# olegroshka/vae-channel-dynamics

Measured on AMD Instinct MI355X. Metric: images/sec SDXL-VAE train step @256x256 (tracking on), higher is better.
Workload: dtype f32

## Files before the change

vae-channel-dynamics_amd/csrc/bf16_frag.h:

```cpp
#pragma once
#include "common.h"

typedef __bf16 bf16x8 __attribute__((ext_vector_type(8)));
typedef __bf16 bf16x4 __attribute__((ext_vector_type(4)));
typedef short s16x4 __attribute__((ext_vector_type(4)));
typedef short s16x8 __attribute__((ext_vector_type(8)));
typedef unsigned short u16;

__device__ __forceinline__ uint2 pack4(f32x4 v) {
  bf16x4 h;
#pragma unroll
  for (int e = 0; e < 4; ++e) h[e] = (__bf16)v[e];
  return __builtin_bit_cast(uint2, h);
}
__device__ __forceinline__ f32x4 unpack4(uint2 r) {
  f32x4 v;
  v[0] = __builtin_bit_cast(float, r.x << 16);
  v[1] = __builtin_bit_cast(float, r.x & 0xffff0000u);
  v[2] = __builtin_bit_cast(float, r.y << 16);
  v[3] = __builtin_bit_cast(float, r.y & 0xffff0000u);
  return v;
}
__device__ __forceinline__ uint4 buf_load4_raw(__amdgpu_buffer_rsrc_t rs, unsigned esize, int eoff) {
  return __builtin_bit_cast(uint4, __builtin_amdgcn_raw_buffer_load_b128(rs, eoff >= 0 ? (unsigned)eoff * esize : BUF_OOB, 0, 0));
}
__device__ __forceinline__ f32x4 raw4_to_f32(uint4 r, bool bf) {
  if (bf) return unpack4(uint2{r.x, r.y});
  return __builtin_bit_cast(f32x4, r);
}
__device__ __forceinline__ float buf_load1_elem(__amdgpu_buffer_rsrc_t rs, bool bf, int eoff) {
  if (bf) return __builtin_bit_cast(float, (unsigned)__builtin_amdgcn_raw_buffer_load_b16(rs, eoff >= 0 ? (unsigned)eoff * 2u : BUF_OOB, 0, 0) << 16);
  return __builtin_bit_cast(float, __builtin_amdgcn_raw_buffer_load_b32(rs, eoff >= 0 ? (unsigned)eoff * 4u : BUF_OOB, 0, 0));
}
__device__ __forceinline__ void buf_store1_elem(__amdgpu_buffer_rsrc_t rs, bool bf, int eoff, float v) {
  if (bf) {
    const __bf16 h = (__bf16)v;
    __builtin_amdgcn_raw_buffer_store_b16(__builtin_bit_cast(unsigned short, h), rs, eoff >= 0 ? (unsigned)eoff * 2u : BUF_OOB, 0, 0);
  } else {
    __builtin_amdgcn_raw_buffer_store_b32(__builtin_bit_cast(unsigned, v), rs, eoff >= 0 ? (unsigned)eoff * 4u : BUF_OOB, 0, 0);
  }
}
__device__ __forceinline__ bf16x8 frag_direct(const u16* p) {
  return __builtin_bit_cast(bf16x8, *reinterpret_cast<const uint4*>(p));
}
__device__ __forceinline__ bf16x8 frag_tr(const u16* p, int ld) {
  typedef __attribute__((address_space(3))) s16x4 lds_s16x4;
  const s16x4 lo = __builtin_amdgcn_ds_read_tr16_b64_v4i16((lds_s16x4*)(p));
  const s16x4 hi = __builtin_amdgcn_ds_read_tr16_b64_v4i16((lds_s16x4*)(p + 4 * ld));
  s16x8 r = {lo[0], lo[1], lo[2], lo[3], hi[0], hi[1], hi[2], hi[3]};
  return __builtin_bit_cast(bf16x8, r);
}
```

vae-channel-dynamics_amd/csrc/igemm.hip:

```cpp
#include "bf16_frag.h"
#include <algorithm>
#include <stdlib.h>
#include <type_traits>

#include "launchers.h"

namespace {

struct LanePos {
  int lr, lh, trq, trp, trh;
};
__device__ __forceinline__ LanePos lane_pos(int lane) { return LanePos{lane & 31, lane >> 5, (lane & 15) >> 2, lane & 3, (lane >> 4) & 1}; }

struct F32 {
  typedef float elem;
  typedef f32x4 raw4;
  typedef f32x4 frag;
  typedef unsigned off_t;
  static constexpr int BK_ROWS = 32, BK_WGRAD = 32;
  static constexpr int KG = 8;
  static constexpr int PAD_K = 4, PAD_T = 4;
  static constexpr bool SETPRIO = true;
  static constexpr bool PAIR16 = false;
  static constexpr int PLANES = 1;
  static constexpr bool LDS_DYNAMIC = false;
  static constexpr bool flag(int32_t) { return false; }

  static __device__ __forceinline__ raw4 load4(__amdgpu_buffer_rsrc_t rs, unsigned, bool ok, int row, int ld, int c) {
    return VAE_BUF_LOAD4(rs, oob_unless(ok, ((unsigned)row * (unsigned)ld + (unsigned)c) * 4u));
  }
  static __device__ __forceinline__ f32x4 to_f32(raw4 r, bool) { return r; }
  static __device__ __forceinline__ void put4(elem* d, f32x4 v, int) { *reinterpret_cast<f32x4*>(d) = v; }
  static __device__ __forceinline__ void put4_stored(elem* d, raw4, f32x4 v, bool, int) { put4(d, v, 0); }
  static __device__ __forceinline__ frag frag_k(const elem* p, int) { return *reinterpret_cast<const f32x4*>(p); }
  static __device__ __forceinline__ frag frag_t(const elem* tile, int ld, int kg, LanePos l, int col0, int) {
    frag v;
#pragma unroll
    for (int j = 0; j < 4; ++j) v[j] = tile[(kg * 8 + l.lh * 4 + j) * ld + col0 + l.lr];
    return v;
  }
  template <int MI, int NI>
  static __device__ __forceinline__ void frags_tt(frag* a, frag* b, const elem* sA, int ldA, int colA, const elem* sB, int ldB, int colB, int kg, LanePos l,
                                                  int, int) {
#pragma unroll
    for (int j = 0; j < 4; ++j) {
      const int k = kg * 8 + l.lh * 4 + j;
#pragma unroll
      for (int mi = 0; mi < MI; ++mi) a[mi][j] = sA[k * ldA + colA + mi * 32 + l.lr];
#pragma unroll
      for (int ni = 0; ni < NI; ++ni) b[ni][j] = sB[k * ldB + colB + ni * 32 + l.lr];
    }
  }
  template <int MI, int NI>
  static __device__ __forceinline__ void mma(f32x16 (&acc)[MI][NI], const frag* a, const frag* b) {
#pragma unroll
    for (int j = 0; j < 4; ++j)
#pragma unroll
      for (int mi = 0; mi < MI; ++mi)
#pragma unroll
        for (int ni = 0; ni < NI; ++ni) acc[mi][ni] = __builtin_amdgcn_mfma_f32_32x32x2f32(a[mi][j], b[ni][j], acc[mi][ni], 0, 0, 0);
  }
  static __device__ __forceinline__ off_t out_off(bool ok, int orow, int ldc, int col) {
    return ok ? ((unsigned)orow * (unsigned)ldc + (unsigned)col) * 4u : BUF_OOB;
  }
  static __device__ __forceinline__ bool inside(off_t o) { return o != BUF_OOB; }
  static __device__ __forceinline__ float load1(__amdgpu_buffer_rsrc_t rs, bool, off_t o) {
    return __builtin_bit_cast(float, __builtin_amdgcn_raw_buffer_load_b32(rs, o, 0, 0));
  }
  static __device__ __forceinline__ void store1(__amdgpu_buffer_rsrc_t rs, bool, off_t o, float v) {
    __builtin_amdgcn_raw_buffer_store_b32(__builtin_bit_cast(unsigned, v), rs, o, 0, 0);
  }
};

struct BF16 {
  typedef u16 elem;
  typedef uint4 raw4;
  typedef bf16x8 frag;
  typedef int off_t;
  static constexpr int BK_ROWS = 64, BK_WGRAD = 32;
  static constexpr int KG = 16;
  static constexpr int PAD_K = 8, PAD_T = 32;
  static constexpr bool SETPRIO = false;
  static constexpr bool PAIR16 = true;
  static constexpr int PLANES = 1;
  static constexpr bool LDS_DYNAMIC = false;
  static __device__ __forceinline__ bool flag(int32_t v) { return v != 0; }

  static __device__ __forceinline__ raw4 load4(__amdgpu_buffer_rsrc_t rs, unsigned esize, bool ok, int row, int ld, int c) {
    return buf_load4_raw(rs, esize, neg_unless(ok, row * ld + c));
  }
  static __device__ __forceinline__ f32x4 to_f32(raw4 r, bool bf) { return raw4_to_f32(r, bf); }
  static __device__ __forceinline__ void put4(elem* d, f32x4 v, int) { *reinterpret_cast<uint2*>(d) = pack4(v); }
  static __device__ __forceinline__ void put4_stored(elem* d, raw4 r, f32x4 v, bool bf, int) {
    *reinterpret_cast<uint2*>(d) = bf ? uint2{r.x, r.y} : pack4(v);
  }
  static __device__ __forceinline__ frag frag_k(const elem* p, int) { return frag_direct(p); }
  static __device__ __forceinline__ frag frag_t(const elem* tile, int ld, int kg, LanePos l, int col0, int) {
    return frag_tr(tile + (kg * 16 + l.lh * 8 + l.trq) * ld + col0 + l.trh * 16 + l.trp * 4, ld);
  }
  template <int MI, int NI>
  static __device__ __forceinline__ void frags_tt(frag* a, frag* b, const elem* sA, int ldA, int colA, const elem* sB, int ldB, int colB, int kg, LanePos l,
                                                  int, int) {
#pragma unroll
    for (int mi = 0; mi < MI; ++mi) a[mi] = frag_t(sA, ldA, kg, l, colA + mi * 32, 0);
#pragma unroll
    for (int ni = 0; ni < NI; ++ni) b[ni] = frag_t(sB, ldB, kg, l, colB + ni * 32, 0);
  }
  template <int MI, int NI>
  static __device__ __forceinline__ void mma(f32x16 (&acc)[MI][NI], const frag* a, const frag* b) {
#pragma unroll
    for (int mi = 0; mi < MI; ++mi)
#pragma unroll
      for (int ni = 0; ni < NI; ++ni) acc[mi][ni] = __builtin_amdgcn_mfma_f32_32x32x16_bf16(a[mi], b[ni], acc[mi][ni], 0, 0, 0);
  }
  static __device__ __forceinline__ off_t out_off(bool ok, int orow, int ldc, int col) { return ok ? orow * ldc + col : -1; }
  static __device__ __forceinline__ bool inside(off_t o) { return o >= 0; }
  static __device__ __forceinline__ float load1(__amdgpu_buffer_rsrc_t rs, bool bf, off_t o) { return buf_load1_elem(rs, bf, o); }
  static __device__ __forceinline__ void store1(__amdgpu_buffer_rsrc_t rs, bool bf, off_t o, float v) { buf_store1_elem(rs, bf, o, v); }

  static __device__ __forceinline__ bool pair16(const vae_igemm_args& p, bool cbf, bool rbf, const char* C) {
    return cbf && (p.N % 2 == 0) && (p.ldc % 2 == 0) && (p.res == nullptr || rbf) && p.track == nullptr && ((reinterpret_cast<uintptr_t>(C) & 3u) == 0);
  }
  template <int MI, int NI, class RowPixel>
  static __device__ __forceinline__ void store_pairs(const vae_igemm_args& p, const f32x16 (&acc)[MI][NI], int ni, __amdgpu_buffer_rsrc_t rsC,
                                                     __amdgpu_buffer_rsrc_t rsR, int col, bool colok, int m0, int trow0, int lh, bool s2c,
                                                     RowPixel row_pixel) {
    const bool odd = col & 1;
    const float b0 = (p.bias && colok) ? p.bias[col & ~1] : 0.f, b1 = (p.bias && colok) ? p.bias[col | 1] : 0.f;
#pragma unroll
    for (int mi = 0; mi < MI; ++mi) {
      unsigned o16[8], rr[8];
#pragma unroll
      for (int j = 0; j < 8; ++j) {
        const int r = 2 * j + (odd ? 1 : 0);
        const int row = trow0 + mi * 32 + (r & 3) + 8 * (r >> 2) + 4 * lh;
        int orow = row;
        if (s2c) {
          int b, y, x;
          row_pixel(row < p.M ? row : m0, b, y, x);
          orow = (b * p.g.Ho + y) * p.g.Wo + x;
        }
        o16[j] = (colok && row < p.M) ? (unsigned)(orow * p.ldc + (col & ~1)) * 2u : BUF_OOB;
        rr[j] = 0u;
      }
      if (p.res) {
#pragma unroll
        for (int j = 0; j < 8; ++j) rr[j] = __builtin_amdgcn_raw_buffer_load_b32(rsR, o16[j], 0, 0);
      }
#pragma unroll
      for (int j = 0; j < 8; ++j) {
        const float a0 = p.alpha * acc[mi][ni][2 * j], a1 = p.alpha * acc[mi][ni][2 * j + 1];
        const float recv = lane_xor1(odd ? a0 : a1);
        typedef __bf16 bf16x2_t __attribute__((ext_vector_type(2)));
        bf16x2_t h;
        h[0] = (__bf16)((odd ? recv : a0) + b0 + __builtin_bit_cast(float, rr[j] << 16));
        h[1] = (__bf16)((odd ? a1 : recv) + b1 + __builtin_bit_cast(float, rr[j] & 0xffff0000u));
        __builtin_amdgcn_raw_buffer_store_b32(__builtin_bit_cast(unsigned, h), rsC, o16[j], 0, 0);
      }
    }
  }
};

#ifndef VAE_FLAT_X3
#define VAE_FLAT_X3 1
#endif
struct F32X3 : F32 {
  typedef u16 elem;
  struct frag { bf16x8 p[3]; };
  static constexpr int BK_ROWS = 16, BK_WGRAD = 16;
  static constexpr int KG = 16;
  static constexpr int PAD_K = 8, PAD_T = 32;
  static constexpr bool SETPRIO = false;
  static constexpr int PLANES = 3;
  static constexpr bool LDS_DYNAMIC = true;

  static __device__ __forceinline__ void put4(elem* d, f32x4 v, int ps) {
    const uint2 hi = pack4(v);
    const f32x4 h = unpack4(hi);
    f32x4 r;
#pragma unroll
    for (int e = 0; e < 4; ++e) r[e] = v[e] - h[e];
    const uint2 mid = pack4(r);
    const f32x4 m = unpack4(mid);
#pragma unroll
    for (int e = 0; e < 4; ++e) r[e] = r[e] - m[e];
    *reinterpret_cast<uint2*>(d) = hi;
    *reinterpret_cast<uint2*>(d + ps) = mid;
    *reinterpret_cast<uint2*>(d + 2 * ps) = pack4(r);
  }
  static __device__ __forceinline__ void put4_stored(elem* d, raw4, f32x4 v, bool, int ps) { put4(d, v, ps); }
  static __device__ __forceinline__ frag frag_k(const elem* p, int ps) {
    frag f;
#pragma unroll
    for (int q = 0; q < 3; ++q) f.p[q] = BF16::frag_k(p + q * ps, 0);
    return f;
  }
  static __device__ __forceinline__ frag frag_t(const elem* tile, int ld, int kg, LanePos l, int col0, int ps) {
    frag f;
#pragma unroll
    for (int q = 0; q < 3; ++q) f.p[q] = BF16::frag_t(tile + q * ps, ld, kg, l, col0, 0);
    return f;
  }
  template <int MI, int NI>
  static __device__ __forceinline__ void frags_tt(frag* a, frag* b, const elem* sA, int ldA, int colA, const elem* sB, int ldB, int colB, int kg, LanePos l,
                                                  int psA, int psB) {
#pragma unroll
    for (int mi = 0; mi < MI; ++mi) a[mi] = frag_t(sA, ldA, kg, l, colA + mi * 32, psA);
#pragma unroll
    for (int ni = 0; ni < NI; ++ni) b[ni] = frag_t(sB, ldB, kg, l, colB + ni * 32, psB);
  }
  template <int MI, int NI>
  static __device__ __forceinline__ void mma(f32x16 (&acc)[MI][NI], const frag* a, const frag* b) {
    constexpr int PA[6] = {0, 2, 1, 0, 1, 0}, PB[6] = {2, 0, 1, 1, 0, 0};
#pragma unroll
    for (int t = 0; t < 6; ++t)
#pragma unroll
      for (int mi = 0; mi < MI; ++mi)
#pragma unroll
        for (int ni = 0; ni < NI; ++ni)
          acc[mi][ni] = __builtin_amdgcn_mfma_f32_32x32x16_bf16(a[mi].p[PA[t]], b[ni].p[PB[t]], acc[mi][ni], 0, 0, 0);
  }
};

template <bool VEC, int WAVES>
using F32For = std::conditional_t<VEC && WAVES == 8 && (VAE_FLAT_X3 != 0), F32X3, F32>;

template <class P, int BM, int BN, bool BKM, int XF>
constexpr int rows_lds_elems() {
  constexpr int BK = P::BK_ROWS;
  return 2 * P::PLANES * (BM * (BK + P::PAD_K) + (BKM ? BK * (BN + P::PAD_T) : BN * (BK + P::PAD_K))) +
         ((XF != VAE_XF_NONE) ? 2 * SS_HALF * (4 / (int)sizeof(typename P::elem)) : 0);
}
template <class P, int BM, int BN, int XF>
constexpr int wgrad_lds_elems() {
  return 2 * P::PLANES * P::BK_WGRAD * (BM + P::PAD_T + BN + P::PAD_T) + ((XF != VAE_XF_NONE) ? 2 * SS_HALF * (4 / (int)sizeof(typename P::elem)) : 0);
}
extern __shared__ __attribute__((aligned(16))) unsigned char lds_dynamic[];

template <int MI, int NI>
__device__ __forceinline__ void zero_acc(f32x16 (&acc)[MI][NI]) {
#pragma unroll
  for (int mi = 0; mi < MI; ++mi)
#pragma unroll
    for (int ni = 0; ni < NI; ++ni)
#pragma unroll
      for (int r = 0; r < 16; ++r) acc[mi][ni][r] = 0.f;
}

template <class P, int BM, int BN, int WM, int WN, bool BKM, bool VEC, int XF>
__device__ __forceinline__ void rows_body(const vae_igemm_args& p) {
  typedef typename P::elem elem;
  constexpr int BK = P::BK_ROWS;
  constexpr int NT = 64 * WM * WN;
  constexpr int KQ = BK / 4;
  constexpr int RP = NT / KQ;
  constexpr int LDA = BK + P::PAD_K;
  constexpr int LDB = BKM ? (BN + P::PAD_T) : (BK + P::PAD_K);
  constexpr int SA = BM * LDA;
  constexpr int SB = BKM ? BK * LDB : BN * LDB;
  constexpr int PL = P::PLANES;
  constexpr int STAGE = PL * (SA + SB);
  constexpr int SS = (XF != VAE_XF_NONE) ? 2 * SS_HALF * (4 / (int)sizeof(elem)) : 0;
  constexpr int TM = BM / WM, TN = BN / WN, MI = TM / 32, NI = TN / 32;
  constexpr int AR = BM / RP;
  constexpr int NQ = BN / 4, KR = NT / NQ;
  constexpr int BR = BKM ? (BK / KR) : (BN / RP);
  static_assert(AR >= 1 && BR >= 1 && TM % 32 == 0 && TN % 32 == 0 && (BK / P::KG == 1 || BK / P::KG == 2 || BK / P::KG == 4), "tile/wave layout");
  static_assert(2 * STAGE + SS == rows_lds_elems<P, BM, BN, BKM, XF>(), "the launcher reserves what the body lays out");
  __shared__ __attribute__((aligned(16))) elem smem_static[P::LDS_DYNAMIC ? 1 : 2 * STAGE + SS];
  elem* const smem = P::LDS_DYNAMIC ? reinterpret_cast<elem*>(lds_dynamic) : smem_static;
  float* sS = reinterpret_cast<float*>(smem + 2 * STAGE);

  const int tid = threadIdx.x, lane = tid & 63, wave = tid >> 6;
  const int wm = wave / WN, wn = wave % WN;
  const LanePos lp = lane_pos(lane);
  const int lr = lp.lr, lh = lp.lh;
  const int tilesN = (p.N + BN - 1) / BN;
  const int tm = blockIdx.x / tilesN, tn = blockIdx.x % tilesN;
  const int m0 = tm * BM, n0 = tn * BN;
  const int z = blockIdx.z;
  const vae_conv_geom g = p.g;
  const SrcMap smap = make_srcmap(g);
  const bool abf = P::flag(p.a_bf16), cbf = P::flag(p.out_bf16), rbf = P::flag(p.res_bf16);
  const unsigned esA = abf ? 2u : 4u;
  const char* __restrict__ A = reinterpret_cast<const char*>(p.A) + (int64_t)z * p.sAb * esA;
  const float* __restrict__ W = p.W + (int64_t)z * p.sWb;
  const int hw = g.Ho * g.Wo;

  const bool s2c = (g.mode == VAE_MODE_DGRAD_S2);
  const int hh = g.Ho >> 1, wh = g.Wo >> 1;
  const int cls_rows = s2c ? p.M >> 2 : 1;
  const int cls = s2c ? m0 / cls_rows : 0;
  const int cpy = cls >> 1, cpx = cls & 1;
  const int nkw = s2c ? (cpx ? 1 : 2) : 3;
  const int ntaps = s2c ? (cpy ? 1 : 2) * nkw : g.taps;
  auto row_pixel = [&](int m, int& b, int& y, int& x) {
    if (s2c) {
      const int r = m - cls * cls_rows;
      b = r / (hh * wh);
      const int rem = r - b * (hh * wh);
      const int i = rem / wh;
      y = 2 * i + cpy;
      x = 2 * (rem - i * wh) + cpx;
    } else {
      b = m / hw;
      const int rem = m - b * hw;
      y = rem / g.Wo;
      x = rem - y * g.Wo;
    }
  };

  const int b_base = s2c ? (m0 - cls * cls_rows) / (hh * wh) : m0 / hw;
  const size_t img = (size_t)g.Hs * g.Ws * g.Cs;
  const size_t abytes = (size_t)(g.B - b_base) * img * esA, wbytes = (size_t)(BKM ? (int64_t)p.K * p.sk : (int64_t)p.N * p.sn) * 4u;
  const auto rsA = VAE_BUF_RSRC(A + (int64_t)b_base * img * esA, abytes < BUF_MAX ? abytes : BUF_MAX);
  const auto rsW = VAE_BUF_RSRC(W, wbytes < BUF_MAX ? wbytes : BUF_MAX);

  const int k4 = tid % KQ, r0 = tid / KQ;
  const int n4 = tid % NQ, kq = tid / NQ;
  int rb[AR], ry[AR], rx[AR];
#pragma unroll
  for (int i = 0; i < AR; ++i) {
    const int m = m0 + r0 + RP * i;
    if (m < p.M) {
      row_pixel(m, rb[i], ry[i], rx[i]);
    } else {
      rb[i] = -1; ry[i] = 0; rx[i] = 0;
    }
  }

  const int b_lo = m0 / hw;
  if (XF != VAE_XF_NONE) {
    const int b_hi = (min(p.M, m0 + BM) - 1) / hw;
    const int nent = min((b_hi - b_lo + 1) * p.K, SS_HALF);
    for (int i = tid; i < nent; i += NT) {
      const int j = i / p.K, c = i - j * p.K;
      sS[i] = p.scale[(int64_t)(b_lo + j) * g.Cs + c];
      sS[SS_HALF + i] = p.shift[(int64_t)(b_lo + j) * g.Cs + c];
    }
  }

  f32x16 acc[MI][NI];
  zero_acc(acc);

  const int kchunks = (p.K + BK - 1) / BK;
  const int steps = ntaps * kchunks;

  typename P::raw4 ra[AR];
  f32x4 rw[BR];
  int a_b[AR];
  int reg_c0 = 0;

  auto load_regs = [&](int s) {
    const int ord = s / kchunks;
    const int c0 = (s - ord * kchunks) * BK;
    reg_c0 = c0;
    int kh, kw;
    if (s2c) {
      const int a = ord / nkw;
      kh = cpy ? 1 : 2 * a;
      kw = cpx ? 1 : 2 * (ord - a * nkw);
    } else {
      kh = (g.taps == 9) ? ord / 3 : 0;
      kw = (g.taps == 9) ? ord - kh * 3 : 0;
    }
    const int tap = kh * 3 + kw;
    const int c = c0 + k4 * 4;
#pragma unroll
    for (int i = 0; i < AR; ++i) {
      int sy = 0, sx = 0;
      const bool ok = src_pixel(smap, ry[i], rx[i], kh, kw, sy, sx) && (rb[i] >= 0);
      if constexpr (VEC) ra[i] = P::load4(rsA, esA, ok && c < p.K, ((rb[i] - b_base) * g.Hs + sy) * g.Ws + sx, g.Cs, c);
      else ra[i] = load4s(p.A + (int64_t)z * p.sAb + (((int64_t)rb[i] * g.Hs + sy) * g.Ws + sx) * g.Cs + c, ok, c, p.K);
      a_b[i] = ok ? rb[i] : -1;
    }
    if (!BKM) {
#pragma unroll
      for (int i = 0; i < BR; ++i) {
        const int n = n0 + r0 + RP * i;
        if constexpr (VEC) rw[i] = VAE_BUF_LOAD4(rsW, oob_unless(n < p.N && c < p.K, ((unsigned)n * (unsigned)p.sn + (unsigned)tap * (unsigned)p.st + (unsigned)c) * 4u));
        else rw[i] = load4s(W + (int64_t)n * p.sn + (int64_t)tap * p.st + c, n < p.N, c, p.K);
      }
    } else {
#pragma unroll
      for (int i = 0; i < BR; ++i) {
        const int k = c0 + kq + KR * i;
        const int n = n0 + n4 * 4;
        if constexpr (VEC) rw[i] = VAE_BUF_LOAD4(rsW, oob_unless(k < p.K && n < p.N, ((unsigned)k * (unsigned)p.sk + (unsigned)tap * (unsigned)p.st + (unsigned)n) * 4u));
        else rw[i] = load4s(W + (int64_t)k * p.sk + (int64_t)tap * p.st + n, k < p.K, n, p.N);
      }
    }
  };
  auto store_lds = [&](elem* sA, elem* sB) {
    const int c = reg_c0 + k4 * 4;
#pragma unroll
    for (int i = 0; i < AR; ++i) {
      f32x4 v = P::to_f32(ra[i], abf);
      if (XF != VAE_XF_NONE) {
        const bool ok = (a_b[i] >= 0) && (c < p.K);
        const int o = ok ? (a_b[i] - b_lo) * p.K + c : 0;
        v = xform4_tab<XF>(v, sS + o, sS + SS_HALF + o, ok);
      }
      P::put4(&sA[(r0 + RP * i) * LDA + k4 * 4], v, SA);
    }
#pragma unroll
    for (int i = 0; i < BR; ++i) {
      if (!BKM) P::put4(&sB[(r0 + RP * i) * LDB + k4 * 4], rw[i], SB);
      else P::put4(&sB[(kq + KR * i) * LDB + n4 * 4], rw[i], SB);
    }
  };
  typename P::frag fa[2][MI], fb[2][NI];
  auto fetch = [&](const elem* sA, const elem* sB, int kg, typename P::frag* a, typename P::frag* b) {
#pragma unroll
    for (int mi = 0; mi < MI; ++mi) a[mi] = P::frag_k(&sA[(wm * TM + mi * 32 + lr) * LDA + kg * P::KG + lh * (P::KG / 2)], SA);
#pragma unroll
    for (int ni = 0; ni < NI; ++ni) {
      if (!BKM) b[ni] = P::frag_k(&sB[(wn * TN + ni * 32 + lr) * LDB + kg * P::KG + lh * (P::KG / 2)], SB);
      else b[ni] = P::frag_t(sB, LDB, kg, lp, wn * TN + ni * 32, SB);
    }
  };
  constexpr int NKG = BK / P::KG;
  auto compute = [&](const elem* sA, const elem* sB, int kg) {
    if (kg + 1 < NKG) fetch(sA, sB, kg + 1, fa[(kg + 1) & 1], fb[(kg + 1) & 1]);
    __builtin_amdgcn_sched_barrier(0);
    if (P::SETPRIO) __builtin_amdgcn_s_setprio(1);
    P::mma(acc, fa[kg & 1], fb[kg & 1]);
    if (P::SETPRIO) __builtin_amdgcn_s_setprio(0);
    __builtin_amdgcn_sched_barrier(0);
  };
  load_regs(0);
  __syncthreads();
  store_lds(smem, smem + PL * SA);
  if (steps > 1) load_regs(1);
  __syncthreads();
  for (int s = 0; s < steps; ++s) {
    const elem* cA = smem + (s & 1) * STAGE;
    const elem* cB = cA + PL * SA;
    fetch(cA, cB, 0, fa[0], fb[0]);
    if (NKG > 1) compute(cA, cB, 0);
    if (NKG == 4) compute(cA, cB, 1);
    if (s + 1 < steps) {
      elem* nA = smem + ((s + 1) & 1) * STAGE;
      store_lds(nA, nA + PL * SA);
      if (s + 2 < steps) load_regs(s + 2);
    }
    compute(cA, cB, NKG / 2);
    if (NKG == 4) compute(cA, cB, 3);
    __syncthreads();
  }

  const unsigned esC = cbf ? 2u : 4u, esR = rbf ? 2u : 4u;
  char* __restrict__ C = reinterpret_cast<char*>(p.C) + (int64_t)z * p.sCb * esC;
  const auto rsC = VAE_BUF_RSRC(C, (size_t)p.M * p.ldc * esC);
  const auto rsR = VAE_BUF_RSRC(p.res ? reinterpret_cast<const char*>(p.res) + (int64_t)z * p.sCb * esR : C, (size_t)p.M * p.ldc * (p.res ? esR : esC));
  float tsum[NI];
#pragma unroll
  for (int ni = 0; ni < NI; ++ni) tsum[ni] = 0.f;
  bool pair16 = false;
  if constexpr (P::PAIR16) pair16 = P::pair16(p, cbf, rbf, C);
#pragma unroll
  for (int ni = 0; ni < NI; ++ni) {
    const int col = n0 + wn * TN + ni * 32 + lr;
    const bool colok = col < p.N;
    const float bv = (p.bias && colok) ? p.bias[col] : 0.f;
    if constexpr (P::PAIR16) {
      if (pair16) {
        P::store_pairs(p, acc, ni, rsC, rsR, col, colok, m0, m0 + wm * TM, lh, s2c, row_pixel);
        continue;
      }
    }
#pragma unroll
    for (int mi = 0; mi < MI; ++mi) {
      typename P::off_t off[16];
      float rv[16];
#pragma unroll
      for (int r = 0; r < 16; ++r) {
        const int row = m0 + wm * TM + mi * 32 + (r & 3) + 8 * (r >> 2) + 4 * lh;
        int orow = row;
        if (s2c) {
          int b, y, x;
          row_pixel(row < p.M ? row : m0, b, y, x);
          orow = (b * g.Ho + y) * g.Wo + x;
        }
        off[r] = P::out_off(colok && row < p.M, orow, p.ldc, col);
        rv[r] = 0.f;
      }
      if (p.res) {
#pragma unroll
        for (int r = 0; r < 16; ++r) rv[r] = P::load1(rsR, rbf, off[r]);
      }
#pragma unroll
      for (int r = 0; r < 16; ++r) {
        const float v = p.alpha * acc[mi][ni][r] + bv + rv[r];
        P::store1(rsC, cbf, off[r], v);
        tsum[ni] += P::inside(off[r]) ? fabsf(v) : 0.f;
      }
    }
  }
  if (p.track && z == 0) {
    float* red = reinterpret_cast<float*>(smem);
#pragma unroll
    for (int ni = 0; ni < NI; ++ni) {
      const float s2 = tsum[ni] + __shfl_xor(tsum[ni], 32, 64);
      if (lh == 0) red[wm * BN + wn * TN + ni * 32 + lr] = s2;
    }
    __syncthreads();
    if (tid < BN) {
      float t = 0.f;
#pragma unroll
      for (int w = 0; w < WM; ++w) t += red[w * BN + tid];
      if (n0 + tid < p.N) p.track[(int64_t)tm * p.N + n0 + tid] = t;
    }
  }
}

template <class P, int BM, int BN, int WM, int WN, bool VEC, int XF>
__device__ __forceinline__ void wgrad_body(const vae_wgrad_args& p) {
  typedef typename P::elem elem;
  constexpr int BK = P::BK_WGRAD;
  constexpr int NT = 64 * WM * WN;
  constexpr int LDA = BM + P::PAD_T, LDB = BN + P::PAD_T;
  constexpr int SA = BK * LDA, SB = BK * LDB;
  constexpr int PL = P::PLANES;
// ... 513 lines not shown
```

vae-channel-dynamics_amd/csrc/wgrad3_wino.hip:

```cpp
#include "wino_common.h"
#ifndef VAE_ABLATE
#define VAE_ABLATE 0
#endif
#ifndef VAE_WGRAD_DEFER
#define VAE_WGRAD_DEFER 2
#endif
#ifndef VAE_WGRAD_PRIO
#define VAE_WGRAD_PRIO 1
#endif
#include <algorithm>
#include <type_traits>

namespace {

constexpr int GCI = 32, GCO = 128, GNT = 512;
constexpr int XS = 20;
constexpr int SXF = 4 * GCI * XS;
constexpr int SYF = 2 * GCO * XS;
constexpr int GSTAGE = SXF + SYF;

template <int XF>
__global__ __launch_bounds__(GNT, 1) void wgrad3_wino_kernel(vae_wgrad_args p, int strips, int64_t nunits) {
  __shared__ __attribute__((aligned(16))) float smem[2 * GSTAGE];

  const int tid = threadIdx.x, lane = tid & 63, wave = tid >> 6;
  const int lr = lane & 31, lh = lane >> 5;
  const vae_conv_geom g = p.g;
  const int tilesN = p.N / GCI, ntile = tilesN * (p.M / GCO);
  const wino::SplitTile wg = wino::split_tile_of_workgroup<true>(blockIdx.x, p.nsplit, ntile);
  const int tile = wg.tile, split = wg.split;
  const int tm = tile / tilesN, tn = tile % tilesN;
  const int m0 = tm * GCO, n0 = tn * GCI;
  const wino::UnitRange ur = wino::unit_range(nunits, p.nsplit, split);
  const int64_t ubeg = ur.ubeg;
  const int nu = ur.nu;
  const int upi = (g.Ho / 2) * strips;
  const bool do_bias = (p.bias_partial != nullptr) && tn == 0;
#ifdef VAE_WGRAD_TIMING
  constexpr int TS0 = 2, TSN = 8;
  const bool tw = (tid & 255) == 0 && blockIdx.x < 8 && p.out != nullptr;
  unsigned long long* const tout = reinterpret_cast<unsigned long long*>(p.out) + (blockIdx.x * 2 + (tid >> 8)) * (4 + TSN * 5);
  unsigned long long tst[5];
  const unsigned long long te0 = __builtin_amdgcn_s_memtime(), tr0 = __builtin_amdgcn_s_memrealtime();
#define GSTAMP(i) do { __builtin_amdgcn_sched_barrier(0); tst[i] = __builtin_amdgcn_s_memtime(); __builtin_amdgcn_sched_barrier(0); } while (0)
#define GSTAMPS_OUT(k) do { if (tw && (k) >= TS0 && (k) < TS0 + TSN) { _Pragma("unroll") for (int i_ = 0; i_ < 5; ++i_) tout[4 + ((k) - TS0) * 5 + i_] = tst[i_]; } } while (0)
#else
#define GSTAMP(i) do { } while (0)
#define GSTAMPS_OUT(k) do { } while (0)
#endif

  const int xx = tid & 15, xq = (tid >> 4) & 7, xr = tid >> 7;
  const bool xe_role = tid < 128 && (tid & 8) == 0;
  const int ex = 16 + (tid & 1), er = (tid >> 1) & 3;
  const int yq = tid >> 4;
  const auto rsX = VAE_BUF_RSRC(p.X, (size_t)g.B * g.Hs * g.Ws * g.Cs * 4u);
  const auto rsY = VAE_BUF_RSRC(p.dY, (size_t)g.B * g.Ho * g.Wo * p.ldy * 4u);
  struct Stg {
    f32x4 rx, rxe, ry[2];
    int b;
    bool xin, xein;
  };
  const f32x4 z4 = {0.f, 0.f, 0.f, 0.f};
  Stg s0{z4, z4, {z4, z4}, -1, false, false}, s1 = s0;
  f32x4 bsum = z4;
  f32x4 rsc = {1.f, 1.f, 1.f, 1.f}, rsh = z4;
  int sc_b = -1;
  int ub = (int)(ubeg / upi), uty = (int)((ubeg - (int64_t)ub * upi) / strips), ustrip = (int)((ubeg - (int64_t)ub * upi) % strips);
  const unsigned thrX = ((xr * g.Ws + xx) * g.Cs + n0 + 4 * xq) * 4u, thrE = ((er * g.Ws + ex) * g.Cs + n0 + 4 * xq) * 4u;
  const unsigned thrY = (xx * p.ldy + m0 + 4 * yq) * 4u, rowY = (unsigned)g.Wo * p.ldy * 4u;
  const int tfX = (xr == 0 ? 1 : 0) | (xr == 3 ? 2 : 0) | (xx == 0 ? 4 : 0) | 16;
  const int tfE = xe_role ? ((er == 0 ? 1 : 0) | (er == 3 ? 2 : 0) | (ex == 17 ? 8 : 0) | 16) : 31;
  auto load_unit = [&](int k, Stg& r) {
    const bool ok = k < nu;
    const int b = ub, ty = uty, x0 = ustrip * 16;
    if (++ustrip == strips) {
      ustrip = 0;
      if (++uty == g.Ho / 2) {
        uty = 0;
        ++ub;
      }
    }
    r.b = ok ? b : -1;
    const int uf = (ty == 0 ? 1 : 0) | (2 * ty + 2 >= g.Hs ? 2 : 0) | (x0 == 0 ? 4 : 0) | (x0 + 16 >= g.Ws ? 8 : 0) | (ok ? 0 : 16);
    const unsigned baseX = (unsigned)((b * g.Hs + 2 * ty - 1) * g.Ws + x0 - 1) * (unsigned)g.Cs * 4u;
    const unsigned baseY = (unsigned)((b * g.Ho + 2 * ty) * g.Wo + x0) * (unsigned)p.ldy * 4u;
    r.xin = (tfX & uf) == 0;
    r.rx = VAE_BUF_LOAD4(rsX, r.xin ? baseX + thrX : BUF_OOB);
    r.xein = (tfE & uf) == 0;
    r.rxe = VAE_BUF_LOAD4(rsX, r.xein ? baseX + thrE : BUF_OOB);
#pragma unroll
    for (int a = 0; a < 2; ++a) r.ry[a] = VAE_BUF_LOAD4(rsY, ok ? baseY + a * rowY + thrY : BUF_OOB);
  };
  auto xform = [&](f32x4 v, bool in) {
    if (XF != VAE_XF_NONE) {
#pragma unroll
      for (int e = 0; e < 4; ++e) {
        float u = v[e] * rsc[e] + rsh[e];
        if (XF == VAE_XF_AFFINE_SILU) u = silu_f(u);
        v[e] = in ? u : 0.f;
      }
    }
    return v;
  };
  auto store_unit = [&](float* st, const Stg& r) {
    float* sx = st;
    float* sy = st + SXF;
    if (XF != VAE_XF_NONE && r.b >= 0 && r.b != sc_b) {
      sc_b = r.b;
      rsc = *reinterpret_cast<const f32x4*>(p.scale + (int64_t)sc_b * g.Cs + n0 + 4 * xq);
      rsh = *reinterpret_cast<const f32x4*>(p.shift + (int64_t)sc_b * g.Cs + n0 + 4 * xq);
    }
    const f32x4 v = xform(r.rx, r.xin);
#pragma unroll
    for (int e = 0; e < 4; ++e) sx[(xr * GCI + 4 * xq + e) * XS + xx] = v[e];
    if (xe_role) {
      const f32x4 ve = xform(r.rxe, r.xein);
#pragma unroll
      for (int e = 0; e < 4; ++e) sx[(er * GCI + 4 * xq + e) * XS + ex] = ve[e];
    }
#pragma unroll
    for (int a = 0; a < 2; ++a) {
#pragma unroll
      for (int e = 0; e < 4; ++e) sy[(a * GCO + 4 * yq + e) * XS + xx] = r.ry[a][e];
      if (do_bias) bsum += r.ry[a];
    }
  };

  const int wi = wave >> 1, jh = wave & 1;
  const int vr1 = wi == 0 ? 0 : (wi == 2 ? 2 : 1), vr2 = wi == 0 ? 2 : (wi == 1 ? 2 : (wi == 2 ? 1 : 3));
  const int voff1 = (vr1 * GCI + lr) * XS + 8 * lh, voff2 = (vr2 * GCI + lr) * XS + 8 * lh;
  const int dr1 = wi == 3 ? 1 : 0;

  f32x16 acc[2][4];
#pragma unroll
  for (int pi = 0; pi < 2; ++pi)
#pragma unroll
    for (int nb = 0; nb < 4; ++nb)
#pragma unroll
      for (int e = 0; e < 16; ++e) acc[pi][nb][e] = 0.f;

  load_unit(0, s0);
  store_unit(smem, s0);
  load_unit(1, s1);
  __syncthreads();

  auto run = [&](auto WI, auto JH) {
    constexpr int wic = decltype(WI)::value, jhc = decltype(JH)::value;
    constexpr bool two = wic == 1 || wic == 2;
    constexpr bool vplus = wic == 1;
    constexpr int ndef = wic >= 2 ? VAE_WGRAD_DEFER : 0;
    static_assert(ndef >= 0 && ndef <= 2, "bb holds the operands of two channel blocks");
    f32x4 a4[2], bb[2][2];
    if (ndef > 0) {
      a4[0] = a4[1] = z4;
      bb[0][0] = bb[0][1] = bb[1][0] = bb[1][1] = z4;
    }
    auto held_back = [&]() {
#pragma unroll
      for (int e = 0; e < 4; ++e)
#pragma unroll
        for (int nb = 4 - ndef; nb < 4; ++nb)
#pragma unroll
          for (int pi = 0; pi < 2; ++pi) acc[pi][nb] = __builtin_amdgcn_mfma_f32_32x32x2f32(a4[pi][e], bb[nb & 1][pi][e], acc[pi][nb], 0, 0, 0);
    };
    auto step = [&](int k, const Stg& cur, Stg& nxt) {
      const float* cx = smem + (k & 1) * GSTAGE;
      const float* cy = cx + SXF;
      float* nst = smem + ((k + 1) & 1) * GSTAGE;
      GSTAMP(0);
      if (ndef > 0) {
        __builtin_amdgcn_sched_barrier(0);
        held_back();
        __builtin_amdgcn_sched_barrier(0);
      }
      GSTAMP(1);
      f32x4 rd[2][2];
      auto read_d = [&](int nb, f32x4 (&d)[2][2]) {
        const int doff = (dr1 * GCO + nb * 32 + lr) * XS + 8 * lh;
#pragma unroll
        for (int c = 0; c < 2; ++c) {
          d[0][c] = *reinterpret_cast<const f32x4*>(&cy[doff + 4 * c]);
          if (two) d[1][c] = *reinterpret_cast<const f32x4*>(&cy[doff + GCO * XS + 4 * c]);
        }
      };
      auto build_b = [&](const f32x4 (&d)[2][2], f32x4 (&b4)[2]) {
        float rc[8];
#pragma unroll
        for (int c = 0; c < 2; ++c)
#pragma unroll
          for (int e = 0; e < 4; ++e) rc[4 * c + e] = !two ? d[0][c][e] : (vplus ? d[0][c][e] + d[1][c][e] : d[0][c][e] - d[1][c][e]);
#pragma unroll
        for (int e = 0; e < 4; ++e) {
          if (jhc == 0) {
            b4[0][e] = rc[2 * e];
            b4[1][e] = rc[2 * e] + rc[2 * e + 1];
          } else {
            b4[0][e] = rc[2 * e] - rc[2 * e + 1];
            b4[1][e] = rc[2 * e + 1];
          }
        }
      };
      {
        f32x4 u1[3], u2[3];
#pragma unroll
        for (int c = 0; c < 3; ++c) {
          u1[c] = *reinterpret_cast<const f32x4*>(&cx[voff1 + 4 * c]);
          u2[c] = *reinterpret_cast<const f32x4*>(&cx[voff2 + 4 * c]);
        }
        float rc[12];
#pragma unroll
        for (int c = 0; c < 3; ++c)
#pragma unroll
          for (int e = 0; e < 4; ++e) rc[4 * c + e] = vplus ? u1[c][e] + u2[c][e] : u1[c][e] - u2[c][e];
        __builtin_amdgcn_sched_barrier(0);
        read_d(0, rd);
#pragma unroll
        for (int e = 0; e < 4; ++e) {
          if (jhc == 0) {
            a4[0][e] = rc[2 * e] - rc[2 * e + 2];
            a4[1][e] = rc[2 * e + 1] + rc[2 * e + 2];
          } else {
            a4[0][e] = rc[2 * e + 2] - rc[2 * e + 1];
            a4[1][e] = rc[2 * e + 1] - rc[2 * e + 3];
          }
        }
        build_b(rd, bb[0]);
        read_d(1, rd);
      }
      if (!(VAE_ABLATE & 2) && wave < 4) store_unit(nst, cur);
      GSTAMP(2);
#pragma unroll
      for (int nb = 0; nb < 4; ++nb) {
        __builtin_amdgcn_sched_barrier(0);
        if (nb == 1) {
          if (!(VAE_ABLATE & 1)) load_unit(k + 2, nxt);
          __builtin_amdgcn_sched_barrier(0);
        }
        if (nb == 3 && wave >= 4) {
          if (!(VAE_ABLATE & 2)) store_unit(nst, cur);
          __builtin_amdgcn_sched_barrier(0);
        }
        if (nb < 3) build_b(rd, bb[(nb + 1) & 1]);
        if (nb < 2) read_d(nb + 2, rd);
        if (nb < 4 - ndef) {
#pragma unroll
          for (int pi = 0; pi < 2; ++pi)
#pragma unroll
            for (int e = 0; e < 4; ++e) acc[pi][nb] = __builtin_amdgcn_mfma_f32_32x32x2f32(a4[pi][e], bb[nb & 1][pi][e], acc[pi][nb], 0, 0, 0);
#pragma unroll
          for (int i = 0; i < 4; ++i) {
            __builtin_amdgcn_sched_group_barrier(0x008, 1, 0);
            __builtin_amdgcn_sched_group_barrier(0x002, 3, 0);
          }
          __builtin_amdgcn_sched_group_barrier(0x100, 4, 0);
          __builtin_amdgcn_sched_group_barrier(0x008, 4, 0);
        }
        __builtin_amdgcn_sched_barrier(0);
        if (nb == 3 - ndef) GSTAMP(3);
      }
      GSTAMP(4);
      GSTAMPS_OUT(k);
      if (!(VAE_ABLATE & 16)) __syncthreads();
    };
    int k = 0;
    for (; k + 1 < nu; k += 2) {
      step(k, s1, s0);
      step(k + 1, s0, s1);
    }
    if (k < nu) step(k, s1, s0);
    if (ndef > 0 && nu > 0) held_back();
  };
#if VAE_WGRAD_PRIO
  if (__builtin_amdgcn_readfirstlane(tid) >= 256) __builtin_amdgcn_s_setprio(1);
#endif
  {
    using J0 = std::integral_constant<int, 0>;
    using J1 = std::integral_constant<int, 1>;
    switch (wave) {
      case 0: run(std::integral_constant<int, 0>{}, J0{}); break;
      case 1: run(std::integral_constant<int, 0>{}, J1{}); break;
      case 2: run(std::integral_constant<int, 1>{}, J0{}); break;
      case 3: run(std::integral_constant<int, 1>{}, J1{}); break;
      case 4: run(std::integral_constant<int, 2>{}, J0{}); break;
      case 5: run(std::integral_constant<int, 2>{}, J1{}); break;
      case 6: run(std::integral_constant<int, 3>{}, J0{}); break;
      default: run(std::integral_constant<int, 3>{}, J1{}); break;
    }
  }
#if VAE_WGRAD_PRIO
  __builtin_amdgcn_s_setprio(0);
#endif

#ifdef VAE_WGRAD_TIMING
  if (tw) {
    tout[0] = te0;
    tout[1] = __builtin_amdgcn_s_memtime();
    tout[2] = tr0;
    tout[3] = __builtin_amdgcn_s_memrealtime();
  }
#endif
  float* __restrict__ O = p.partial + (int64_t)split * 16 * p.N * p.M;
  wino::slab_store<4>(O, wi * 4 + 2 * jh, p.N, p.M, n0, m0, 0, acc[0], lr, lh);
  wino::slab_store<4>(O, wi * 4 + 2 * jh + 1, p.N, p.M, n0, m0, 0, acc[1], lr, lh);
  if (do_bias) wino::bias_tail(bsum, xx, p.bias_partial, (int64_t)split * p.M + m0 + 4 * yq);
}

}

bool wgrad3_wino_eligible(const vae_wgrad_args& a) {
  const vae_conv_geom& g = a.g;
  if (!wino::wgrad_eligible_common(a, GCI, GCO) || g.mode != VAE_MODE_FWD || g.Ho != g.Hs || g.Wo != g.Ws) return false;
  return g.Ho % 2 == 0 && g.Wo % 16 == 0;
}

int64_t wgrad3_wino_units(const vae_conv_geom& g) { return (int64_t)g.B * (g.Ho / 2) * (g.Wo / 16); }

int launch_wgrad3_wino(const vae_wgrad_args& a, hipStream_t st) {
  const vae_conv_geom& g = a.g;
  const int64_t nunits = wgrad3_wino_units(g);
  dim3 grid((unsigned)((a.M / GCO) * (a.N / GCI) * a.nsplit), 1, 1);
  const int strips = g.Wo / 16;
  dispatch_xf_or_silu(a.xf, [&](auto xf) { hipLaunchKernelGGL(wgrad3_wino_kernel<decltype(xf)::value>, grid, dim3(GNT), 0, st, a, strips, nunits); });
  return 0;
}
```

Before: 109.4.

## Switch Winograd wgrad kernel to bf16x3 split MFMA with paired double-buffered stages

Adds a new default wgrad3_wino kernel variant that splits the Winograd-transformed f32 operands into three bf16 planes and accumulates six bf16 32x32x16 MFMA terms, emulating f32 precision on the bf16 matrix cores. Each iteration now stages two units per double-buffer slot in dynamically reserved LDS. Shared helpers for the 3-way split (using paired vector bf16 conversion) and the MFMA term are factored into bf16_frag.h and reused by the existing igemm F32X3 path. The aim is higher matrix throughput than the previous f32 path, at the cost of extra split arithmetic, register pressure, and slightly different rounding.

```diff
diff --git a/vae-channel-dynamics_amd/csrc/bf16_frag.h b/vae-channel-dynamics_amd/csrc/bf16_frag.h
--- a/vae-channel-dynamics_amd/csrc/bf16_frag.h
+++ b/vae-channel-dynamics_amd/csrc/bf16_frag.h
@@ -20,6 +20,28 @@
   v[2] = __builtin_bit_cast(float, r.y << 16);
   v[3] = __builtin_bit_cast(float, r.y & 0xffff0000u);
   return v;
+}
+__device__ __forceinline__ uint2 pack4_pairs(f32x4 v) {
+  typedef float f32x2_t __attribute__((ext_vector_type(2)));
+  typedef __bf16 bf16x2_t __attribute__((ext_vector_type(2)));
+  const f32x2_t a = {v[0], v[1]}, b = {v[2], v[3]};
+  return uint2{__builtin_bit_cast(unsigned, __builtin_convertvector(a, bf16x2_t)), __builtin_bit_cast(unsigned, __builtin_convertvector(b, bf16x2_t))};
+}
+__device__ __forceinline__ void split3(f32x4 v, uint2& hi, uint2& mid, uint2& lo) {
+  hi = pack4_pairs(v);
+  const f32x4 h = unpack4(hi);
+  f32x4 r;
+#pragma unroll
+  for (int e = 0; e < 4; ++e) r[e] = v[e] - h[e];
+  mid = pack4_pairs(r);
+  const f32x4 m = unpack4(mid);
+#pragma unroll
+  for (int e = 0; e < 4; ++e) r[e] = r[e] - m[e];
+  lo = pack4_pairs(r);
+}
+__device__ __forceinline__ f32x16 mma_x3_term(int t, const bf16x8 (&a)[3], const bf16x8 (&b)[3], f32x16 acc) {
+  constexpr int PA[6] = {0, 2, 1, 0, 1, 0}, PB[6] = {2, 0, 1, 1, 0, 0};
+  return __builtin_amdgcn_mfma_f32_32x32x16_bf16(a[PA[t]], b[PB[t]], acc, 0, 0, 0);
 }
 __device__ __forceinline__ uint4 buf_load4_raw(__amdgpu_buffer_rsrc_t rs, unsigned esize, int eoff) {
   return __builtin_bit_cast(uint4, __builtin_amdgcn_raw_buffer_load_b128(rs, eoff >= 0 ? (unsigned)eoff * esize : BUF_OOB, 0, 0));
diff --git a/vae-channel-dynamics_amd/csrc/igemm.hip b/vae-channel-dynamics_amd/csrc/igemm.hip
--- a/vae-channel-dynamics_amd/csrc/igemm.hip
+++ b/vae-channel-dynamics_amd/csrc/igemm.hip
@@ -175,18 +175,11 @@
   static constexpr bool LDS_DYNAMIC = true;
 
   static __device__ __forceinline__ void put4(elem* d, f32x4 v, int ps) {
-    const uint2 hi = pack4(v);
-    const f32x4 h = unpack4(hi);
-    f32x4 r;
-#pragma unroll
-    for (int e = 0; e < 4; ++e) r[e] = v[e] - h[e];
-    const uint2 mid = pack4(r);
-    const f32x4 m = unpack4(mid);
-#pragma unroll
-    for (int e = 0; e < 4; ++e) r[e] = r[e] - m[e];
+    uint2 hi, mid, lo;
+    split3(v, hi, mid, lo);
     *reinterpret_cast<uint2*>(d) = hi;
     *reinterpret_cast<uint2*>(d + ps) = mid;
-    *reinterpret_cast<uint2*>(d + 2 * ps) = pack4(r);
+    *reinterpret_cast<uint2*>(d + 2 * ps) = lo;
   }
   static __device__ __forceinline__ void put4_stored(elem* d, raw4, f32x4 v, bool, int ps) { put4(d, v, ps); }
   static __device__ __forceinline__ frag frag_k(const elem* p, int ps) {
@@ -211,14 +204,12 @@
   }
   template <int MI, int NI>
   static __device__ __forceinline__ void mma(f32x16 (&acc)[MI][NI], const frag* a, const frag* b) {
-    constexpr int PA[6] = {0, 2, 1, 0, 1, 0}, PB[6] = {2, 0, 1, 1, 0, 0};
 #pragma unroll
     for (int t = 0; t < 6; ++t)
 #pragma unroll
       for (int mi = 0; mi < MI; ++mi)
 #pragma unroll
-        for (int ni = 0; ni < NI; ++ni)
-          acc[mi][ni] = __builtin_amdgcn_mfma_f32_32x32x16_bf16(a[mi].p[PA[t]], b[ni].p[PB[t]], acc[mi][ni], 0, 0, 0);
+        for (int ni = 0; ni < NI; ++ni) acc[mi][ni] = mma_x3_term(t, a[mi].p, b[ni].p, acc[mi][ni]);
   }
 };
 
diff --git a/vae-channel-dynamics_amd/csrc/wgrad3_wino.hip b/vae-channel-dynamics_amd/csrc/wgrad3_wino.hip
--- a/vae-channel-dynamics_amd/csrc/wgrad3_wino.hip
+++ b/vae-channel-dynamics_amd/csrc/wgrad3_wino.hip
@@ -7,6 +7,12 @@
 #endif
 #ifndef VAE_WGRAD_PRIO
 #define VAE_WGRAD_PRIO 1
+#endif
+#ifndef VAE_WGRAD_X3
+#define VAE_WGRAD_X3 1
+#endif
+#if VAE_WGRAD_X3
+#include "bf16_frag.h"
 #endif
 #include <algorithm>
 #include <type_traits>
@@ -19,6 +25,7 @@
 constexpr int SYF = 2 * GCO * XS;
 constexpr int GSTAGE = SXF + SYF;
 
+#if !VAE_WGRAD_X3
 template <int XF>
 __global__ __launch_bounds__(GNT, 1) void wgrad3_wino_kernel(vae_wgrad_args p, int strips, int64_t nunits) {
   __shared__ __attribute__((aligned(16))) float smem[2 * GSTAGE];
@@ -305,6 +312,296 @@
   if (do_bias) wino::bias_tail(bsum, xx, p.bias_partial, (int64_t)split * p.M + m0 + 4 * yq);
 }
 
+#else
+constexpr int GPAIR = 2 * GSTAGE;
+constexpr int GLDS = 2 * GPAIR * (int)sizeof(float);
+extern __shared__ __attribute__((aligned(16))) float wgrad_lds[];
+
+struct Bf3 {
+  bf16x8 p[3];
+};
+__device__ __forceinline__ Bf3 split8(f32x4 v0, f32x4 v1) {
+  uint2 q0[3], q1[3];
+  split3(v0, q0[0], q0[1], q0[2]);
+  split3(v1, q1[0], q1[1], q1[2]);
+  Bf3 f;
+#pragma unroll
+  for (int i = 0; i < 3; ++i) f.p[i] = __builtin_bit_cast(bf16x8, uint4{q0[i].x, q0[i].y, q1[i].x, q1[i].y});
+  return f;
+}
+
+template <int XF>
+__global__ __launch_bounds__(GNT, 1) void wgrad3_wino_kernel(vae_wgrad_args p, int strips, int64_t nunits) {
+  float* const smem = wgrad_lds;
+
+  const int tid = threadIdx.x, lane = tid & 63, wave = tid >> 6;
+  const int lr = lane & 31, lh = lane >> 5;
+  const vae_conv_geom g = p.g;
+  const int tilesN = p.N / GCI, ntile = tilesN * (p.M / GCO);
+  const wino::SplitTile wg = wino::split_tile_of_workgroup<true>(blockIdx.x, p.nsplit, ntile);
+  const int tile = wg.tile, split = wg.split;
+  const int tm = tile / tilesN, tn = tile % tilesN;
+  const int m0 = tm * GCO, n0 = tn * GCI;
+  const wino::UnitRange ur = wino::unit_range(nunits, p.nsplit, split);
+  const int64_t ubeg = ur.ubeg;
+  const int nu = ur.nu;
+  const int upi = (g.Ho / 2) * strips;
+  const bool do_bias = (p.bias_partial != nullptr) && tn == 0;
+#ifdef VAE_WGRAD_TIMING
+  constexpr int TS0 = 2, TSN = 8;
+  const bool tw = (tid & 255) == 0 && blockIdx.x < 8 && p.out != nullptr;
+  unsigned long long* const tout = reinterpret_cast<unsigned long long*>(p.out) + (blockIdx.x * 2 + (tid >> 8)) * (4 + TSN * 5);
+  unsigned long long tst[5];
+  const unsigned long long te0 = __builtin_amdgcn_s_memtime(), tr0 = __builtin_amdgcn_s_memrealtime();
+#define GSTAMP(i) do { __builtin_amdgcn_sched_barrier(0); tst[i] = __builtin_amdgcn_s_memtime(); __builtin_amdgcn_sched_barrier(0); } while (0)
+#define GSTAMPS_OUT(k) do { if (tw && (k) >= TS0 && (k) < TS0 + TSN) { _Pragma("unroll") for (int i_ = 0; i_ < 5; ++i_) tout[4 + ((k) - TS0) * 5 + i_] = tst[i_]; } } while (0)
+#else
+#define GSTAMP(i) do { } while (0)
+#define GSTAMPS_OUT(k) do { } while (0)
+#endif
+
+  const int xx = tid & 15, xq = (tid >> 4) & 7, xr = tid >> 7;
+  const bool xe_role = tid < 128 && (tid & 8) == 0;
+  const int ex = 16 + (tid & 1), er = (tid >> 1) & 3;
+  const int yq = tid >> 4;
+  const auto rsX = VAE_BUF_RSRC(p.X, (size_t)g.B * g.Hs * g.Ws * g.Cs * 4u);
+  const auto rsY = VAE_BUF_RSRC(p.dY, (size_t)g.B * g.Ho * g.Wo * p.ldy * 4u);
+  const auto rsS = VAE_BUF_RSRC(p.scale, (size_t)g.B * g.Cs * 4u);
+  const auto rsH = VAE_BUF_RSRC(p.shift, (size_t)g.B * g.Cs * 4u);
+  struct Stg {
+    f32x4 rx, rxe, ry[2];
+    int b, uf;
+  };
+  const f32x4 z4 = {0.f, 0.f, 0.f, 0.f};
+  Stg s0{z4, z4, {z4, z4}, -1, 16}, s1 = s0;
+  f32x4 bsum = z4;
+  f32x4 rsc = {1.f, 1.f, 1.f, 1.f}, rsh = z4;
+  int sc_b = -1;
+  int ub = (int)(ubeg / upi), uty = (int)((ubeg - (int64_t)ub * upi) / strips), ustrip = (int)((ubeg - (int64_t)ub * upi) % strips);
+  const unsigned thrX = ((xr * g.Ws + xx) * g.Cs + n0 + 4 * xq) * 4u, thrE = ((er * g.Ws + ex) * g.Cs + n0 + 4 * xq) * 4u;
+  const unsigned thrY = (xx * p.ldy + m0 + 4 * yq) * 4u, rowY = (unsigned)g.Wo * p.ldy * 4u;
+  const int tfX = (xr == 0 ? 1 : 0) | (xr == 3 ? 2 : 0) | (xx == 0 ? 4 : 0) | 16;
+  const int tfE = xe_role ? ((er == 0 ? 1 : 0) | (er == 3 ? 2 : 0) | (ex == 17 ? 8 : 0) | 16) : 31;
+  auto load_unit = [&](int k, Stg& r) __attribute__((always_inline)) {
+    const bool ok = k < nu;
+    const int b = ub, ty = uty, x0 = ustrip * 16;
+    if (++ustrip == strips) {
+      ustrip = 0;
+      if (++uty == g.Ho / 2) {
+        uty = 0;
+        ++ub;
+      }
+    }
+    r.b = ok ? b : -1;
+    const int uf = (ty == 0 ? 1 : 0) | (2 * ty + 2 >= g.Hs ? 2 : 0) | (x0 == 0 ? 4 : 0) | (x0 + 16 >= g.Ws ? 8 : 0) | (ok ? 0 : 16);
+    const unsigned baseX = (unsigned)((b * g.Hs + 2 * ty - 1) * g.Ws + x0 - 1) * (unsigned)g.Cs * 4u;
+    const unsigned baseY = (unsigned)((b * g.Ho + 2 * ty) * g.Wo + x0) * (unsigned)p.ldy * 4u;
+    r.uf = uf;
+    r.rx = VAE_BUF_LOAD4(rsX, (tfX & uf) == 0 ? baseX + thrX : BUF_OOB);
+    r.rxe = VAE_BUF_LOAD4(rsX, (tfE & uf) == 0 ? baseX + thrE : BUF_OOB);
+#pragma unroll
+    for (int a = 0; a < 2; ++a) r.ry[a] = VAE_BUF_LOAD4(rsY, ok ? baseY + a * rowY + thrY : BUF_OOB);
+  };
+  auto xform = [&](f32x4 v, bool in) {
+    if (XF != VAE_XF_NONE) {
+#pragma unroll
+      for (int e = 0; e < 4; ++e) {
+        float u = v[e] * rsc[e] + rsh[e];
+        if (XF == VAE_XF_AFFINE_SILU) u = silu_f(u);
+        v[e] = in ? u : 0.f;
+      }
+    }
+    return v;
+  };
+  auto store_unit = [&](float* st, const Stg& r) __attribute__((always_inline)) {
+    float* sx = st;
+    float* sy = st + SXF;
+    if (XF != VAE_XF_NONE && r.b >= 0 && r.b != sc_b) {
+      sc_b = r.b;
+      const unsigned at = (unsigned)(sc_b * g.Cs + n0 + 4 * xq) * 4u;
+      rsc = VAE_BUF_LOAD4(rsS, at);
+      rsh = VAE_BUF_LOAD4(rsH, at);
+    }
+    const f32x4 v = xform(r.rx, (tfX & r.uf) == 0);
+#pragma unroll
+    for (int e = 0; e < 4; ++e) sx[(xr * GCI + 4 * xq + e) * XS + xx] = v[e];
+    if (xe_role) {
+      const f32x4 ve = xform(r.rxe, (tfE & r.uf) == 0);
+#pragma unroll
+      for (int e = 0; e < 4; ++e) sx[(er * GCI + 4 * xq + e) * XS + ex] = ve[e];
+    }
+#pragma unroll
+    for (int a = 0; a < 2; ++a) {
+#pragma unroll
+      for (int e = 0; e < 4; ++e) sy[(a * GCO + 4 * yq + e) * XS + xx] = r.ry[a][e];
+      if (do_bias) bsum += r.ry[a];
+    }
+  };
+  auto stage_pair = [&](float* st, int kp) __attribute__((always_inline)) {
+    if (!(VAE_ABLATE & 2)) {
+      store_unit(st, s0);
+      store_unit(st + GSTAGE, s1);
+    }
+    if (!(VAE_ABLATE & 1)) {
+      load_unit(2 * kp + 2, s0);
+      load_unit(2 * kp + 3, s1);
+    }
+  };
+
+  const int wi = wave >> 1, jh = wave & 1;
+  const int vr1 = wi == 0 ? 0 : (wi == 2 ? 2 : 1), vr2 = wi == 0 ? 2 : (wi == 1 ? 2 : (wi == 2 ? 1 : 3));
+  const int voff1 = (vr1 * GCI + lr) * XS + 8 * lh, voff2 = (vr2 * GCI + lr) * XS + 8 * lh;
+  const int dr1 = wi == 3 ? 1 : 0;
+
+  f32x16 acc[2][4];
+#pragma unroll
+  for (int pi = 0; pi < 2; ++pi)
+#pragma unroll
+    for (int nb = 0; nb < 4; ++nb)
+#pragma unroll
+      for (int e = 0; e < 16; ++e) acc[pi][nb][e] = 0.f;
+
+  load_unit(0, s0);
+  load_unit(1, s1);
+  stage_pair(smem, 0);
+  __syncthreads();
+  const int np = (nu + 1) / 2;
+
+  auto run = [&](auto WI, auto JH) {
+    constexpr int wic = decltype(WI)::value, jhc = decltype(JH)::value;
+    constexpr bool two = wic == 1 || wic == 2;
+    constexpr bool vplus = wic == 1;
+    Bf3 a3[2], bb[2];
+    auto mma = [&](auto NB) {
+      constexpr int nb = decltype(NB)::value;
+#pragma unroll
+      for (int t = 0; t < 6; ++t)
+#pragma unroll
+        for (int pi = 0; pi < 2; ++pi) acc[pi][nb] = mma_x3_term(t, a3[pi].p, bb[pi].p, acc[pi][nb]);
+    };
+    auto step = [&](int kp) {
+      const float* cst = smem + (kp & 1) * GPAIR;
+      float* nst = smem + ((kp + 1) & 1) * GPAIR;
+      GSTAMP(0);
+      GSTAMP(1);
+      {
+        f32x4 af[2][2];
+#pragma unroll
+        for (int u = 0; u < 2; ++u) {
+          const float* cx = cst + u * GSTAGE;
+          f32x4 u1[3], u2[3];
+#pragma unroll
+          for (int c = 0; c < 3; ++c) {
+            u1[c] = *reinterpret_cast<const f32x4*>(&cx[voff1 + 4 * c]);
+            u2[c] = *reinterpret_cast<const f32x4*>(&cx[voff2 + 4 * c]);
+          }
+          float rc[12];
+#pragma unroll
+          for (int c = 0; c < 3; ++c)
+#pragma unroll
+            for (int e = 0; e < 4; ++e) rc[4 * c + e] = vplus ? u1[c][e] + u2[c][e] : u1[c][e] - u2[c][e];
+#pragma unroll
+          for (int e = 0; e < 4; ++e) {
+            if (jhc == 0) {
+              af[u][0][e] = rc[2 * e] - rc[2 * e + 2];
+              af[u][1][e] = rc[2 * e + 1] + rc[2 * e + 2];
+            } else {
+              af[u][0][e] = rc[2 * e + 2] - rc[2 * e + 1];
+              af[u][1][e] = rc[2 * e + 1] - rc[2 * e + 3];
+            }
+          }
+        }
+#pragma unroll
+        for (int pi = 0; pi < 2; ++pi) a3[pi] = split8(af[0][pi], af[1][pi]);
+      }
+      if (wic < 2) stage_pair(nst, kp + 1);
+      __builtin_amdgcn_sched_barrier(0);
+      auto block = [&](auto NB) {
+        constexpr int nb = decltype(NB)::value;
+        if (nb == 3 && wic >= 2) {
+          __builtin_amdgcn_sched_barrier(0);
+          stage_pair(nst, kp + 1);
+          __builtin_amdgcn_sched_barrier(0);
+        }
+        f32x4 bf[2][2];
+#pragma unroll
+        for (int u = 0; u < 2; ++u) {
+          const float* cy = cst + u * GSTAGE + SXF;
+          const int doff = (dr1 * GCO + nb * 32 + lr) * XS + 8 * lh;
+          f32x4 d[2][2];
+#pragma unroll
+          for (int c = 0; c < 2; ++c) {
+            d[0][c] = *reinterpret_cast<const f32x4*>(&cy[doff + 4 * c]);
+            if (two) d[1][c] = *reinterpret_cast<const f32x4*>(&cy[doff + GCO * XS + 4 * c]);
+          }
+          float rc[8];
+#pragma unroll
+          for (int c = 0; c < 2; ++c)
+#pragma unroll
+            for (int e = 0; e < 4; ++e) rc[4 * c + e] = !two ? d[0][c][e] : (vplus ? d[0][c][e] + d[1][c][e] : d[0][c][e] - d[1][c][e]);
+#pragma unroll
+          for (int e = 0; e < 4; ++e) {
+            if (jhc == 0) {
+              bf[u][0][e] = rc[2 * e];
+              bf[u][1][e] = rc[2 * e] + rc[2 * e + 1];
+            } else {
+              bf[u][0][e] = rc[2 * e] - rc[2 * e + 1];
+              bf[u][1][e] = rc[2 * e + 1];
+            }
+          }
+        }
+#pragma unroll
+        for (int pi = 0; pi < 2; ++pi) bb[pi] = split8(bf[0][pi], bf[1][pi]);
+        if (nb == 0) GSTAMP(2);
+        mma(NB);
+        if (nb == 3) GSTAMP(3);
+      };
+      block(std::integral_constant<int, 0>{});
+      block(std::integral_constant<int, 1>{});
+      block(std::integral_constant<int, 2>{});
+      block(std::integral_constant<int, 3>{});
+      GSTAMP(4);
+      GSTAMPS_OUT(kp);
+      if (!(VAE_ABLATE & 16)) __syncthreads();
+    };
+    for (int kp = 0; kp < np; ++kp) step(kp);
+  };
+#if VAE_WGRAD_PRIO
+  if (__builtin_amdgcn_readfirstlane(tid) >= 256) __builtin_amdgcn_s_setprio(1);
+#endif
+  {
+    using J0 = std::integral_constant<int, 0>;
+    using J1 = std::integral_constant<int, 1>;
+    switch (wave) {
+      case 0: run(std::integral_constant<int, 0>{}, J0{}); break;
+      case 1: run(std::integral_constant<int, 0>{}, J1{}); break;
+      case 2: run(std::integral_constant<int, 1>{}, J0{}); break;
+      case 3: run(std::integral_constant<int, 1>{}, J1{}); break;
+      case 4: run(std::integral_constant<int, 2>{}, J0{}); break;
+      case 5: run(std::integral_constant<int, 2>{}, J1{}); break;
+      case 6: run(std::integral_constant<int, 3>{}, J0{}); break;
+      default: run(std::integral_constant<int, 3>{}, J1{}); break;
+    }
+  }
+#if VAE_WGRAD_PRIO
+  __builtin_amdgcn_s_setprio(0);
+#endif
+
+#ifdef VAE_WGRAD_TIMING
+  if (tw) {
+    tout[0] = te0;
+    tout[1] = __builtin_amdgcn_s_memtime();
+    tout[2] = tr0;
+    tout[3] = __builtin_amdgcn_s_memrealtime();
+  }
+#endif
+  float* __restrict__ O = p.partial + (int64_t)split * 16 * p.N * p.M;
+  wino::slab_store<4>(O, wi * 4 + 2 * jh, p.N, p.M, n0, m0, 0, acc[0], lr, lh);
+  wino::slab_store<4>(O, wi * 4 + 2 * jh + 1, p.N, p.M, n0, m0, 0, acc[1], lr, lh);
+  if (do_bias) wino::bias_tail(bsum, xx, p.bias_partial, (int64_t)split * p.M + m0 + 4 * yq);
+}
+#endif
+
 }
 
 bool wgrad3_wino_eligible(const vae_wgrad_args& a) {
@@ -320,6 +617,16 @@
   const int64_t nunits = wgrad3_wino_units(g);
   dim3 grid((unsigned)((a.M / GCO) * (a.N / GCI) * a.nsplit), 1, 1);
   const int strips = g.Wo / 16;
+#if VAE_WGRAD_X3
+  int rc = 0;
+  dispatch_xf_or_silu(a.xf, [&](auto xf) {
+    constexpr int XF = decltype(xf)::value;
+    rc = [&]() -> int { VAE_RESERVE_LDS(wgrad3_wino_kernel<XF>, GLDS, "wgrad3_wino"); return 0; }();
+    if (rc == 0) hipLaunchKernelGGL(wgrad3_wino_kernel<XF>, grid, dim3(GNT), GLDS, st, a, strips, nunits);
+  });
+  return rc;
+#else
   dispatch_xf_or_silu(a.xf, [&](auto xf) { hipLaunchKernelGGL(wgrad3_wino_kernel<decltype(xf)::value>, grid, dim3(GNT), 0, st, a, strips, nunits); });
   return 0;
+#endif
 }
```

After: 112.9 (median of 6 runs). 3.1% higher.
